# ablab/stringdecomposer

Hardware: AMD Instinct MI355X
Metric: decomposed read-bp/sec (whole node) at 12 monomers x 50kb reads (higher is better)
Workload: dtype u16

## Files before the change

include/sd_hip.h:

```cpp
#ifndef SD_HIP_H
#define SD_HIP_H

#include <stddef.h>
#include <stdint.h>

#ifdef __cplusplus
extern "C" {
#endif

#define SD_OK 0
#define SD_ERR_IO 2
#define SD_ERR_FORMAT 3
#define SD_ERR_PARAM 4
#define SD_ERR_EMPTY 6
#define SD_ERR_INTERNAL 7
#define SD_ERR_NO_DEVICE 8
#define SD_ERR_UNSUPPORTED 9
#define SD_ERR_HIP 10
#define SD_ERR_SYMBOL 255

typedef struct sd_params {
    int32_t ins, del, mismatch, match;
    int32_t part_size;
    int32_t overlap;
// ... 149 lines not shown

int sd_engine_load_reads(sd_engine* e, const char* const* read_seqs, const int64_t* read_lens,
                         int32_t n_reads, int64_t* n_chunks, char* errbuf, size_t errlen);

int sd_engine_load_reads_dev(sd_engine* e, const void* d_bases, const int64_t* read_off, const int64_t* read_lens,
                             int32_t n_reads, void* hip_stream, int64_t* n_chunks, char* errbuf, size_t errlen);

int sd_engine_run(sd_engine* e, void* hip_stream, char* errbuf, size_t errlen);

int sd_engine_fetch(sd_engine* e, sd_rec** recs, int64_t** rec_off, char* errbuf, size_t errlen);

int sd_engine_assemble(sd_engine* e, const sd_rec* recs, const int64_t* rec_off, sd_rec** rows,
                       int64_t** row_off, char* errbuf, size_t errlen);

int sd_engine_rows_dev(sd_engine* e, sd_rec* d_rows, int64_t cap_rows, int64_t* d_row_off, void* hip_stream, int64_t* n_rows,
                       char* errbuf, size_t errlen);

int sd_engine_timings(sd_engine* e, float ms[4]);

int sd_engine_info(sd_engine* e, int64_t info[8]);

int sd_plan_info(const sd_params* p, const char* const* mono_seqs, const int32_t* mono_lens, int32_t n_mono,
                 int64_t info[8], char* errbuf, size_t errlen);

typedef struct sd_stream sd_stream;
int sd_stream_create(sd_stream** out, const sd_params* p, const char* const* mono_seqs,
                     const int32_t* mono_lens, int32_t n_mono, int32_t sub_batches, char* errbuf,
                     size_t errlen);
void sd_stream_destroy(sd_stream* s);
int sd_stream_submit(sd_stream* s, const char* const* read_seqs, const int64_t* read_lens,
                     int32_t n_reads, char* errbuf, size_t errlen);
int sd_stream_submit_dev(sd_stream* s, const void* d_bases, const int64_t* read_off, const int64_t* read_lens,
                         int32_t n_reads, void* hip_stream, char* errbuf, size_t errlen);
int sd_stream_collect(sd_stream* s, sd_rec** rows, int64_t** row_off, int64_t* n_rows, char* errbuf,
                      size_t errlen);
int sd_stream_peek_dev(sd_stream* s, int32_t* n_reads, int64_t* max_rows, char* errbuf, size_t errlen);
int sd_stream_collect_dev(sd_stream* s, sd_rec* d_rows, int64_t cap_rows, int64_t* d_row_off, void* hip_stream,
                          int64_t* n_rows, char* errbuf, size_t errlen);
int sd_stream_stats(sd_stream* s, double out[16]);
int sd_stream_info(sd_stream* s, int64_t info[8]);

typedef struct sd_final_row {
    int32_t read;
    int64_t start, end;
    int32_t best, second, homo_best, homo_second;
    double ident, second_ident, homo_ident, homo_second_ident;
// ... 112 lines not shown
```

stringdecomposer_amd/csrc/sd_engine.hip:

```cpp
#include <hip/hip_runtime.h>

#include <fcntl.h>
#include <unistd.h>

#include <algorithm>
#include <atomic>
#include <condition_variable>
#include <deque>
#include <mutex>
#include <chrono>
#include <functional>
#include <cstdlib>
#include <cstring>
#include <memory>
#include <string>
#include <thread>
#include <vector>

#include "../../include/sd_hip.h"
#include "sd_convert.hpp"
#include "sd_ident.hpp"
#include "sd_nw.hpp"
#include "sd_device.hpp"
#include "sd_fast.hpp"
// ... 1066 lines not shown
        const int64_t L = (int64_t)e.tseq[j].size();
        int64_t run = 0, lanes_seen = 0;
        for (int64_t k = 0; k < L; ++k, ++x) {
            const uint32_t so = plan.slot_of[(size_t)x];
            const bool new_lane = k == 0 || (so & 127u) != (plan.slot_of[(size_t)x - 1] & 127u) || (so >> 16) != (plan.slot_of[(size_t)x - 1] >> 16);
            if (new_lane && k > 0) {
                if (lanes_seen == 0) min_first = std::min(min_first, run);
                max_lane = std::max(max_lane, run);
                ++lanes_seen;
                run = 0;
            }
            ++run;
        }
        if (lanes_seen == 0) min_first = std::min(min_first, run);
        max_lane = std::max(max_lane, run);
    }
    info[5] = min_first;
    info[6] = max_lane;
    info[7] = (int64_t)e.score_scale | ((int64_t)(plan.tr2_ok ? plan.tr2_qm : 0) << 16) | ((int64_t)(plan.tr2_ok ? plan.tr2_bound : 0) << 24) |
              ((int64_t)((plan.Hx >> 8) & 1) << 56);
    return SD_OK;
}

int sd_engine_create(sd_engine** out, const sd_params* p, const char* const* mono_seqs,
                     const int32_t* mono_lens, int32_t n_mono, char* errbuf, size_t errlen) {
    if (!out) return SD_ERR_PARAM;
    *out = nullptr;
    std::string err;
    int rc = validate_params(p, err);
    if (rc) { set_err(errbuf, errlen, err); return rc; }
    if (n_mono <= 0) { set_err(errbuf, errlen, "no monomers"); return SD_ERR_PARAM; }
    std::unique_ptr<sd_engine> e(new sd_engine);
    e->p = *p;
    apply_env_overrides(e->p);
    rc = host_templates(e.get(), *p, mono_seqs, mono_lens, n_mono, err);
    if (rc) { set_err(errbuf, errlen, err); return rc; }
    {
        const int w0 = (e->tlen[0] - 1) >> 6, h0 = ((e->tlen[0] - 1) >> 5) & 1;
        bool same = true;
        for (int j = 1; j < e->T; ++j) same = same && ((e->tlen[j] - 1) >> 6) == w0 && (((e->tlen[j] - 1) >> 5) & 1) == h0;
        e->filter_uniform = same && w0 == ((e->Lmax + 63) / 64) - 1 ? h0 : -1;
        if (e->p.reserved[1] & SD_FLAG_FILTER_GENERAL) e->filter_uniform = -1;
    }
    rc = check_score_range(*p, e->Lmax, err);
    if (rc) { set_err(errbuf, errlen, err); return rc; }

// ... 540 lines not shown
```

stringdecomposer_amd/csrc/sd_fast.hip:

```cpp
#include <hip/hip_runtime.h>

#include <algorithm>
#include <climits>
#include <cstdlib>
#include <type_traits>

#include "sd_fast.hpp"
#include "sd_fast_dev.hpp"
#include "sd_fast_launch.hpp"

namespace sd {

#ifndef SD_TRACE_MINW
#define SD_TRACE_MINW 7
#endif
#ifndef SD_TRACE_ADAPT
#define SD_TRACE_ADAPT 1
#endif
constexpr int trace_waves_per_group(int QK) { return QK <= 8 ? 4 : 1; }

template <int QK>
__global__ __launch_bounds__(64 * trace_waves_per_group(QK), (QK <= 4 ? SD_TRACE_MINW : QK <= 8 ? 2 : 1)) void sd_fast_trace(
    const ChunkDesc* __restrict__ chunks, int n_chunks, const uint32_t* __restrict__ bases2,
    const uint32_t* __restrict__ nmask, const uint32_t* __restrict__ slot_of,
// ... 425 lines not shown
            Bounds b2;
            const int fs = layout_for(c.first, b2);
            const int ops = cell_ops(c.first, fs);
            if (ops < best) { best = ops; P = c.first; split = c.second; plan.floor_slots = fs; bnd.swap(b2); }
        }
        plan.P = P;
        plan.P4 = (P + 3) & ~3;
    }
    for (int b = 0; b < 5; ++b) plan.floor_sym[b] = 1;
    plan.table_nonneg = std::min(sc.match, sc.mismatch) - sc.del - sc.ins >= 0;
    if (!plan.filter_only)
        for (int j = 0; j < T; ++j) {
            const std::string& sq = tseq[(size_t)j];
            const std::vector<int>& bj = bnd[(size_t)j];
            for (size_t u = 0; u + 1 < bj.size(); ++u)
                for (int b = 0; b < 5; ++b) {
                    int run = code_of(sq[(size_t)bj[u]]) == b ? sc.match : sc.mismatch;
                    for (int q = 1; bj[u] + q < bj[u + 1]; ++q) {
                        const int val = code_of(sq[(size_t)(bj[u] + q)]) == b ? sc.match : sc.mismatch;
                        if (val > run) { run = val; plan.floor_sym[b] = std::max(plan.floor_sym[b], q); }
                    }
                }
        }
    if (getenv("SD_PLAN_DEBUG"))
        std::fprintf(stderr, "[sd plan] P = %d: floor slots %d; per read symbol A C G T N: %d %d %d %d %d\n", P, plan.floor_slots,
                     plan.floor_sym[0], plan.floor_sym[1], plan.floor_sym[2], plan.floor_sym[3], plan.floor_sym[4]);
    plan.T = T;
    plan.split = split;
    plan.Lmax = Lmax;
    plan.Qk = (Lmax + 63) / 64;
    if (plan.Qk == 5) plan.Qk = 6;
    if (plan.Qk == 7) plan.Qk = 8;
    if (plan.Qk > 8) plan.Qk = plan.Qk <= 16 ? 16 : 32;
    plan.vlane0.assign((size_t)T, 0);
    int Vmax = 1;
    if (plan.tiled) {
        for (int j = 0; j < T; ++j) {
            plan.vlane0[(size_t)j] = tiled_v0[(size_t)j];
            Vmax = std::max(Vmax, ((int)tseq[(size_t)j].size() + P - 1) / P);
        }
        plan.bshift = 10;
    } else if (W > 1) {
        for (int j = 0; j < T; ++j) plan.vlane0[(size_t)j] = j;
        plan.bshift = 10;
    } else {
        int v = 0;
        for (int j = 0; j < T; ++j) {
            if (j == split) v = 64;
            plan.vlane0[(size_t)j] = v;
// ... 145 lines not shown
            plan.slot_of[(size_t)x] = (uint32_t)((slot << 7) | v);
            for (int b = 0; b < 5; ++b) {
                const int val = (cd == b ? sc.match : sc.mismatch) - sc.del - sc.ins;
                uint32_t& w = plan.table[(((size_t)b * (P4 / 4) + slot / 4) * 64 + lane) * 4 + (slot & 3)];
                put(w, plane, val);
            }
        }
    }
    if (allow_tr2) fast_plan_trace2(tseq, sc, plan);
    plan.ok = true;
    return true;
}

int64_t fast_ckpt_rows_total(const FastPlan& plan, std::vector<ChunkDesc>& chunks) {
    (void)plan;
    int64_t tot = 0;
    for (ChunkDesc& cd : chunks) {
        cd.pad = (uint32_t)tot;
        tot += (cd.n - 1) / FAST_R;
    }
    return tot;
}

uint32_t fast_fill_hx(const FastPlan& plan, int fl, int step) {
    uint32_t hx = plan.Hx;
    if (step > 0)
        for (int b = 0; b < 5; ++b) {
            uint32_t lv = 0;
            while (lv < 3 && fl - (int)(lv + 1) * step >= std::max(1, plan.floor_sym[b])) ++lv;
            hx |= lv << (22 + 2 * b);
        }
    return hx;
}

template <int... L> static int floor_level(const FastPlan& plan, PList<L...>) {
    for (int c : {L...})
        if (plan.floor_slots >= 1 && plan.floor_slots <= c && c + 2 < plan.P) return c;
    return 0;
}

static int multi_wave_fl(const FastPlan& plan) {
    return !plan.full_floor && floor_level(plan, PList<48>()) ? 48 : plan.P;
}

static void launch_fast_fill_full(const FastPlan& plan, hipStream_t st, const FillArgs& a, int grid, int nw, size_t lds, bool one) {
    with_p(FastP(), plan.P, [&](auto p) {
        constexpr int P = decltype(p)::value;
        with_bool(one, [&](auto on) {
            if (plan.f16) launch_narrow<P, CF_F16, P, decltype(on)::value, 0>(st, a, grid, nw, lds, plan.Hx);
            else launch_narrow<P, CF_I16, P, decltype(on)::value, 0>(st, a, grid, nw, lds, plan.Hx);
        });
    });
}

void launch_fast_fill(const FastPlan& plan, hipStream_t st, const FillArgs& a, size_t min_lds) {
// ... 71 lines not shown
```

stringdecomposer_amd/csrc/sd_fast.hpp:

```cpp
#pragma once

#include <hip/hip_runtime.h>

#include <cstdint>
#include <string>
#include <type_traits>
#include <vector>

#include "sd_device.hpp"

namespace sd {

constexpr int FAST_R = 32;
constexpr int FAST_REBASE = 128;
constexpr int FAST_LANE_WORDS = 8;

enum FastLaneConst {
    FLC_STARTMASK = 0,
    FLC_CONTMASK,
    FLC_ENDOFF,
    FLC_ROW0,
    FLC_TMPL,
    FLC_CONT2,
    FLC_ENDALL,
// ... 4 lines not shown
    bool ok = false;
    bool wide = false;
    bool f16 = false;
    bool u16 = false;
    int u16_lim = 0;
    int P = 0;
    int P4 = 0;
    int H = 0;
    uint32_t Hx = 0;
    int T = 0;
    int split = 0;
    int Lmax = 0;
    int Qk = 0;
    int waves = 1;
    bool tiled = false;
    bool filter_only = false;
    int bshift = 7;
    int rebase = FAST_REBASE;
    int range_bound = 0;
    bool full_floor = false;
    int floor_slots = 0;
    int floor_sym[5] = {0, 0, 0, 0, 0};
    bool table_nonneg = false;
    uint32_t bf8_match = 0, bf8_mismatch = 0;
    std::vector<int32_t> vlane0;
    std::vector<uint32_t> table;
    std::vector<uint32_t> lane_consts;
    std::vector<uint32_t> slot_of;
    std::vector<uint8_t> tcodes;
    std::vector<int32_t> end_vlane;
    std::vector<int32_t> end_off;
    bool tr2_ok = false;
    int tr2_qm = 0;
    int tr2_xlim = 0;
    int tr2_bound = 0;
    std::vector<uint32_t> tr2_tab;
};

void fast_plan_trace2(const std::vector<std::string>& tseq, ScoreArgs sc, FastPlan& plan);

inline bool fast_has_1bp(const FastPlan& plan) { return (plan.Hx >> 10) & 1; }

template <int... Vs> struct PList { static constexpr int v[] = {Vs...}; };
template <int... Vs, typename F> void with_p(PList<Vs...>, int v, F&& f) {
    (void)((v == Vs && (f(std::integral_constant<int, Vs>()), true)) || ...);
}
// ... 81 lines not shown
    const uint8_t* tcodes;
    const uint32_t* lane_consts;
    const int32_t* toff;
    const int32_t* tlen;
    ScoreArgs sc;
    const int32_t* B;
    const int32_t* argV;
    const uint32_t* ckpt;
    const int32_t* ckbase;
    DevRec* recs;
    int32_t* rec_cnt;
    int* queue;
    const int* order;
    int n_cu;
    const uint32_t* tr2_tab = nullptr;
    const uint16_t* klist = nullptr;
    const uint16_t* kpos = nullptr;
    const int32_t* nkept = nullptr;
    const uint32_t* lane_t = nullptr;
};

void launch_fast_fill(const FastPlan& plan, hipStream_t st, const FillArgs& a, size_t min_lds = 0);
void launch_fast_fill_compact(const FastPlan& plan, hipStream_t st, const FillArgs& a, int wb);
uint32_t fast_fill_hx(const FastPlan& plan, int fl, int step);

void launch_fast_fill_fl(const FastPlan& plan, hipStream_t st, const FillArgs& a, int grid, int nw, size_t lds, int fl);
void launch_fast_fill_fl_long(const FastPlan& plan, hipStream_t st, const FillArgs& a, int grid, int nw, size_t lds, int fl);
void launch_fast_fill_fl_u16(const FastPlan& plan, hipStream_t st, const FillArgs& a, int grid, int nw, size_t lds, int fl);
void launch_fast_fill_fl_long_u16(const FastPlan& plan, hipStream_t st, const FillArgs& a, int grid, int nw, size_t lds, int fl);
void launch_fast_fill_fl_u16s(const FastPlan& plan, hipStream_t st, const FillArgs& a, int grid, int nw, size_t lds, int fl);
void launch_fast_fill_fl_long_u16s(const FastPlan& plan, hipStream_t st, const FillArgs& a, int grid, int nw, size_t lds, int fl);
void launch_fast_fill_fl_i16(const FastPlan& plan, hipStream_t st, const FillArgs& a, int grid, int nw, size_t lds, int fl);
void launch_fast_fill_full_u16(const FastPlan& plan, hipStream_t st, const FillArgs& a, int grid, int nw, size_t lds, bool one);
void launch_fast_fill_wide(const FastPlan& plan, hipStream_t st, const FillArgs& a, int grid, size_t lds);
void launch_fast_fill_wide_fl(const FastPlan& plan, hipStream_t st, const FillArgs& a, int grid, size_t lds, int fl);
void launch_fast_fill_wn(const FastPlan& plan, hipStream_t st, const FillArgs& a, int grid, size_t lds);
void launch_fast_fill_wn_fl(const FastPlan& plan, hipStream_t st, const FillArgs& a, int grid, size_t lds);
void launch_fast_fill_wt(const FastPlan& plan, hipStream_t st, const FillArgs& a, int grid, size_t lds, int fl);
void launch_fast_fill_wn_i16(const FastPlan& plan, hipStream_t st, const FillArgs& a, int grid, size_t lds);
void launch_fast_fill_wt_i16(const FastPlan& plan, hipStream_t st, const FillArgs& a, int grid, size_t lds);
void launch_fast_fill_wn_compact(const FastPlan& plan, hipStream_t st, const FillArgs& a, int grid, int wb, size_t lds, int fl);
void launch_fast_fill_wt_compact(const FastPlan& plan, hipStream_t st, const FillArgs& a, int grid, int wb, size_t lds, int fl);

void launch_fast_trace(const FastPlan& plan, hipStream_t st, const TraceArgs& a);
void launch_fast_trace2(const FastPlan& plan, hipStream_t st, const TraceArgs& a);

}
// ... 1 lines not shown
```

stringdecomposer_amd/csrc/sd_fast_fill.hpp:

```cpp
#pragma once

#include <hip/hip_runtime.h>

#include <algorithm>
#include <climits>
#include <cstdlib>
#include <type_traits>

#include "sd_fast.hpp"
#include "sd_fast_dev.hpp"

namespace sd {

#define SD_FILL_NW_MAX 16
template <int P, bool RANKED, int CF, int FL = P, bool ONE = false, int FLS = 0>
__global__ __launch_bounds__(SD_FILL_NW_MAX * 64, 4) void sd_fast_fill(
    const ChunkDesc* __restrict__ chunks, int n_chunks, const uint32_t* __restrict__ bases2,
    const uint32_t* __restrict__ nmask, const uint32_t* __restrict__ table,
    const uint32_t* __restrict__ lane_consts, ScoreArgs sc, int Hx, int32_t* __restrict__ Bout,
    int32_t* __restrict__ argV, uint32_t* __restrict__ ckpt, int32_t* __restrict__ ckbase,
    int* __restrict__ queue, const int* __restrict__ order, const uint32_t* __restrict__ cendoff,
    const uint32_t* __restrict__ crank) {
    constexpr int P4 = (P + 3) & ~3;
    extern __shared__ __attribute__((aligned(16))) uint32_t lds[];
    constexpr int TBL = 5 * P4 * 64;
    constexpr bool F16 = CF == CF_F16, U16 = CF == CF_U16;
    using CO = CellOps<CF>;
    constexpr uint32_t NEGC = CO::NEG;
    for (int idx = threadIdx.x * 4; idx < TBL; idx += blockDim.x * 4) {
        uint4 q = *reinterpret_cast<const uint4*>(&table[idx]);
        if constexpr (F16) {
            q.x = CO::from_i16x2(q.x); q.y = CO::from_i16x2(q.y);
            q.z = CO::from_i16x2(q.z); q.w = CO::from_i16x2(q.w);
        }
        if constexpr (U16) {
            const uint32_t tm = lane_consts[((idx >> 2) & 63) * FAST_LANE_WORDS + FLC_TMPL];
            const int tpad = min(min(sc.match, sc.mismatch) - sc.del - sc.ins, 0);
            const int plo = (tm & 0xffffu) == 0xffffu ? 0 : tpad, phi = (tm >> 16) == 0xffffu ? 0 : tpad;
            auto cv = [&](uint32_t w) {
                const int lo = (int)(short)(w & 0xffffu), hi = (int)w >> 16;
                return spair(lo <= -30000 ? plo : lo, hi <= -30000 ? phi : hi);
            };
            q.x = cv(q.x); q.y = cv(q.y); q.z = cv(q.z); q.w = cv(q.w);
        }
        *reinterpret_cast<uint4*>(&lds[idx]) = q;
    }
    __syncthreads();

    const int wave = __builtin_amdgcn_readfirstlane((int)(threadIdx.x >> 6));
    const int nw = (int)(blockDim.x >> 6);
    const int lane = threadIdx.x & 63;
    (void)wave; (void)nw;
    const int H = Hx & 0xff;
    const bool bperm_ok = (Hx >> 8) & 1;
    FairShare fair;
    fair.init(reinterpret_cast<int*>(lds + TBL), wave, nw, lane, queue, n_chunks);
    ChunkSched sched;
    sched.init(queue, order, n_chunks);
    for (int c = sched.next(); c >= 0; c = sched.next()) {
    const ChunkDesc cd = chunks[c];
    const int n = cd.n;
    ReadStream rs;
    rs.init(bases2 + cd.woff, cd.noff >= 0 ? nmask + cd.noff : nullptr, n);
    bool bperm_scan = bperm_ok && (!fair.drained || ((Hx >> 9) & 1));

    const uint32_t* lc = lane_consts + lane * FAST_LANE_WORDS;
    const uint32_t startMask = lc[FLC_STARTMASK];
    const uint32_t contMask = lc[FLC_CONTMASK];
    const uint32_t cont2Mask = lc[FLC_CONT2];
    const uint32_t oneMask = ONE ? lc[FLC_ONE] : 0u;
    const uint32_t endOffPlan = lc[FLC_ENDOFF];
    constexpr bool HRED = F16 || U16;
    const uint32_t endOffRaw = pk_adds(RANKED ? cendoff[(size_t)c * 64 + lane] : lc[FLC_ENDALL], pack2(sc.del));
    const uint32_t endOff = HRED ? CO::from_i16x2(endOffRaw)
                                 : CO::from_i16x2(RANKED ? cendoff[(size_t)c * 64 + lane] : endOffPlan);
// ... 13 lines not shown
    int32_t* ckb = ckbase + cd.pad;

    uint32_t L[P];
    uint32_t tb[P4];
    uint32_t K = NEGC;
    int base = 0, Brel = 0, tp = 0;
    uint32_t bdel16 = 0;
    int accBV = 0;
    int flush_at = min(n, 64);

    typedef uint32_t u32x4_t __attribute__((ext_vector_type(4)));
    using lds_u4 = __attribute__((address_space(3))) const u32x4_t;
    const uint32_t lds_lane = (uint32_t)(uintptr_t)(__attribute__((address_space(3))) const uint32_t*)lds + lane * 16;
    auto load_table = [&](int r, uint32_t& after) {
        uint32_t addr = lds_lane + (uint32_t)(r * (P4 * 256));
        asm volatile("" : "+v"(addr), "+v"(after));
        lds_u4* t = (lds_u4*)(uintptr_t)addr;
#pragma unroll
        for (int c4 = 0; c4 < P4 / 4; ++c4) {
            const u32x4_t q = t[c4 * 64];
            tb[4 * c4 + 0] = q.x; tb[4 * c4 + 1] = q.y; tb[4 * c4 + 2] = q.z; tb[4 * c4 + 3] = q.w;
        }
    };
    const int idle4 = (Hx >> 16) << 2;
    int bp1 = (contMask & 0xffffu) ? (lane - 1) << 2 : idle4;
    int bp2 = (cont2Mask & 0xffffu) ? (lane - 2) << 2 : idle4;
    asm volatile("" : "+v"(bp1), "+v"(bp2));
    auto excl_scan = [&](uint32_t a) {
        uint32_t inc = a;
        if (bperm_scan) {
            inc = CO::mx(inc, (uint32_t)__builtin_amdgcn_ds_bpermute(bp1, (int)inc));
            inc = CO::mx(inc, (uint32_t)__builtin_amdgcn_ds_bpermute(bp2, (int)inc));
            return (uint32_t)__builtin_amdgcn_ds_bpermute(bp1, (int)inc);
        }
        if (H <= 4) {
            inc = CO::mx(inc, bfi(contMask, lane_up(inc, 1), NEGC));
            inc = CO::mx(inc, bfi(cont2Mask, lane_up(lane_up(inc, 1), 1), NEGC));
        } else {
            for (int h = 1; h < H; ++h) inc = CO::mx(a, bfi(contMask, lane_up(inc, 1), NEGC));
        }
        return bfi(contMask, lane_up(inc, 1), NEGC);
    };
    auto reduce_ends = [&](uint32_t Eend, int row) {
        if constexpr (HRED) {
            uint32_t val = CO::add(Eend, endOff);
            if constexpr (U16 && RANKED) val &= endMask;
            uint32_t m;
// ... 61 lines not shown
        const int v = mlo ? (__ffsll((long long)mlo) - 1) : (64 + __ffsll((long long)mhi) - 1);
        Brel = b + tp * sc.ins;
        const int slot = (row - 1) & 63;
        acc_put(accBV, (int)(((uint32_t)(base + Brel) << 7) | (uint32_t)v), slot);
        if (row == flush_at) {
            flush_at = min(n, row + 64);
            if (lane <= slot) Bc[row - slot + lane] = accBV;
        }
    };

    uint32_t pin = 0;
    load_table(rs.code(0), pin);
    rs.advance(0);
    if constexpr (U16) {
        L[0] = (tb[0] + row0adj + U16_BIAS2) & planeMask;
#pragma unroll
        for (int q = 1; q < P; ++q) L[q] = CO::mx(L[q - 1], (tb[q] + ins2 + U16_BIAS2) & planeMask);
    } else {
    L[0] = CO::add(tb[0], row0adj);
#pragma unroll
    for (int q = 1; q < P; ++q) L[q] = CO::mx(L[q - 1], CO::add(tb[q], ins2));
    }
    int rcur = rs.code(1);
    load_table(rcur, L[P - 1]);
    rs.advance(1);
    std::conditional_t<U16, U16Guard<P>, F16Guard<P>> guard;
    if constexpr (F16) {
        guard.start(L[P - 1], sc.guard_lim);
        guard.check_low(L);
    }
    if constexpr (U16) {
        guard.start(sc.guard_lim);
        guard.check_low(L, planeMask);
    }
    const uint32_t a0 = ONE ? bfi(oneMask, L[0], L[P - 1]) : L[P - 1];
    if constexpr (HRED) reduce_ends(a0, 1);
    K = excl_scan(a0);
    uint32_t Eend = CO::mx(a0, K);
    if constexpr (!HRED) reduce_ends(Eend, 1);

    for (int i = 1; i < n;) {
        if ((i & (FAST_R - 1)) == 0) {
            fair.update(n - i);
            bperm_scan = bperm_ok && (!fair.drained || ((Hx >> 9) & 1));
            if ((i & (127 >> ((Hx >> 11) & 1))) == 0) {
                if constexpr (F16)
// ... 33 lines not shown
            }
            const int q = (i / FAST_R) - 1;
#pragma unroll
            for (int s = 0; s < P; ++s) ck[(uint64_t)q * (P * 64) + s * 64] = CO::mx(L[s], K);
            if (lane == 0) ckb[q] = base + tp * sc.ins;
        }
        const int iend = min(n, (i | (FAST_R - 1)) + 1);
        for (; i < iend; ++i) {
        uint32_t KB;
        if constexpr (HRED) {
            asm("v_pk_max_f16 %0, %1, %2 op_sel_hi:[1,0]" : "=v"(KB) : "v"(K), "s"(bdel16));
            if constexpr (U16) KB &= planeMask;
        } else {
            KB = CO::mx(K, CO::splat(Brel + sc.del - tp * sc.ins));
        }
        const uint32_t w0 = U16 ? (L[0] & notStart) : bfi(startMask, NEGC, L[0]);
        uint32_t u_[P], v_[P], c_[P];
        uint32_t run = 0;
        if constexpr (HRED) {
            if constexpr (FLS > 0) {
                constexpr int FL3 = FL - 3 * FLS > 1 ? FL - 3 * FLS : 1;
                constexpr int FL2 = FL - 2 * FLS > FL3 ? FL - 2 * FLS : FL3;
                constexpr int FL1 = FL - FLS > FL2 ? FL - FLS : FL2;
                const int lv = (Hx >> (22 + 2 * rcur)) & 3;
#pragma unroll
                for (int q = 1; q <= FL3 && q < P; ++q) L[q - 1] = CO::mx(L[q - 1], KB);
                if (lv <= 2) {
#pragma unroll
                    for (int q = FL3 + 1; q <= FL2 && q < P; ++q) L[q - 1] = CO::mx(L[q - 1], KB);
                }
                if (lv <= 1) {
#pragma unroll
                    for (int q = FL2 + 1; q <= FL1 && q < P; ++q) L[q - 1] = CO::mx(L[q - 1], KB);
                }
                if (lv == 0) {
#pragma unroll
                    for (int q = FL1 + 1; q <= FL && q < P; ++q) L[q - 1] = CO::mx(L[q - 1], KB);
                }
            }
            const uint32_t w0f = FLS > 0 ? (U16 ? (L[0] & notStart) : bfi(startMask, NEGC, L[0])) : w0;
#pragma unroll
            for (int s = 0; s < P + 4; ++s) {
                if (s >= 4) {
                    const int q = s - 4;
                    L[q] = q == 0 ? CO::mx3(v_[0], w0f, K) : CO::mx3(L[q - 1], v_[q], L[q]);
                }
                if (s >= 2 && s - 2 < P) {
// ... 12 lines not shown
        } else {
#pragma unroll
        for (int s = 0; s < P + 3; ++s) {
            if (s >= 3) {
                const int q = s - 3;
                run = q == 0 ? c_[0] : pk_max(run, c_[q]);
                L[q] = run;
            }
            if (s >= 2 && s - 2 < P) {
                const int q = s - 2;
                c_[q] = pk_max(v_[q], q == 0 ? w0 : L[q]);
            }
            if (s >= 1 && s - 1 < P) {
                const int q = s - 1;
                v_[q] = pk_adds(u_[q], tb[q]);
            }
            if (s < P) {
                const int q = s;
                u_[q] = q == 0 ? KB : q <= FL ? pk_max(L[q - 1], KB) : L[q - 1];
            }
            __builtin_amdgcn_sched_barrier(0);
        }
        }
        rcur = rs.code(i + 1);
        load_table(rcur, L[P - 1]);
        rs.advance(i + 1);
        uint32_t a = HRED ? L[P - 1] : CO::mx(L[P - 1], K);
        if constexpr (ONE) a = bfi(oneMask, L[0], a);
        ++tp;
        if constexpr (HRED) {
            uint32_t t1 = 0;
            if (bperm_scan) t1 = (uint32_t)__builtin_amdgcn_ds_bpermute(bp1, (int)a);
            reduce_ends(a, i + 1);
            if (bperm_scan) {
                const uint32_t i1 = CO::mx(a, t1);
                const uint32_t i2 = CO::mx(i1, (uint32_t)__builtin_amdgcn_ds_bpermute(bp2, (int)i1));
                K = (uint32_t)__builtin_amdgcn_ds_bpermute(bp1, (int)i2);
            } else {
                K = excl_scan(a);
            }
        } else {
            K = excl_scan(a);
            Eend = CO::mx(a, K);
            reduce_ends(Eend, i + 1);
        }
        }
// ... 12 lines not shown
```

stringdecomposer_amd/csrc/sd_fast_fl.hip:

```cpp
#include "sd_fast_launch.hpp"

#ifndef SD_FL_CF
#define SD_FL_CF CF_F16
#define SD_FL_STEP 0
#define SD_FL_ENTRY launch_fast_fill_fl
#endif

namespace sd {

void SD_FL_ENTRY(const FastPlan& plan, hipStream_t st, const FillArgs& a, int grid, int nw, size_t lds, int fl) {
    const uint32_t hx = fast_fill_hx(plan, fl, SD_FL_STEP);
    with_p(FastFlP(), plan.P, [&](auto p) {
        with_p(FlLevels(), fl, [&](auto f) {
            launch_narrow<decltype(p)::value, SD_FL_CF, decltype(f)::value, false, SD_FL_STEP>(st, a, grid, nw, lds, hx);
        });
    });
}

}
```

stringdecomposer_amd/csrc/sd_fast_fl_long.hip:

```cpp
#include "sd_fast_launch.hpp"

#ifndef SD_FL_CF
#define SD_FL_CF CF_F16
#define SD_FL_STEP 0
#define SD_FL_ENTRY launch_fast_fill_fl_long
#endif

namespace sd {

void SD_FL_ENTRY(const FastPlan& plan, hipStream_t st, const FillArgs& a, int grid, int nw, size_t lds, int fl) {
    const uint32_t hx = fast_fill_hx(plan, fl, SD_FL_STEP);
    with_p(FastFlLongP(), plan.P, [&](auto p) {
        with_p(FlLongLevels(), fl, [&](auto f) {
            launch_narrow<decltype(p)::value, SD_FL_CF, decltype(f)::value, false, SD_FL_STEP>(st, a, grid, nw, lds, hx);
        });
    });
}

}
```

stringdecomposer_amd/csrc/sd_fast_launch.hpp:

```cpp
#pragma once

#include "sd_fast_fill.hpp"
#include "sd_fast_wide_fill.hpp"
#include "sd_fast_wn_fill.hpp"

namespace sd {

template <int P, int CF, int FL, bool ONE, int FLS>
void launch_narrow(hipStream_t st, const FillArgs& a, int grid, int nw, size_t lds, uint32_t hx) {
    with_bool(a.cendoff != nullptr, [&](auto rk) {
        constexpr bool RK = decltype(rk)::value;
        (void)hipFuncSetAttribute(reinterpret_cast<const void*>(&sd_fast_fill<P, RK, CF, FL, ONE, FLS>),
                                  hipFuncAttributeMaxDynamicSharedMemorySize, (int)lds);
        hipLaunchKernelGGL((sd_fast_fill<P, RK, CF, FL, ONE, FLS>), dim3(grid), dim3(nw * 64), lds, st, a.chunks, a.n_chunks,
                           a.bases2, a.nmask, a.table, a.lane_consts, a.sc, (int)hx, a.B, a.argV, a.ckpt, a.ckbase, a.queue,
                           a.order, a.cendoff, a.crank);
    });
}

template <int P, bool F16, int FL>
void launch_wide(hipStream_t st, const FillArgs& a, int grid, size_t lds) {
    with_bool(a.cendoff != nullptr, [&](auto rk) {
        constexpr bool RK = decltype(rk)::value;
        (void)hipFuncSetAttribute(reinterpret_cast<const void*>(&sd_fast_fill_wide<P, RK, F16, FL>),
                                  hipFuncAttributeMaxDynamicSharedMemorySize, (int)lds);
        hipLaunchKernelGGL((sd_fast_fill_wide<P, RK, F16, FL>), dim3(grid), dim3(512), lds, st, a.chunks, a.n_chunks, a.bases2,
                           a.nmask, a.table, a.lane_consts, a.sc, a.B, a.ckpt, a.ckbase, a.queue, a.order, a.cendoff, a.crank);
    });
}

template <int P, int FL, bool COMPACT, bool TILED, bool F16>
void launch_wn(const FastPlan& plan, hipStream_t st, const FillArgs& a, int grid, int nw, size_t lds) {
    auto go = [&](auto rk) {
        constexpr bool RK = decltype(rk)::value;
        (void)hipFuncSetAttribute(reinterpret_cast<const void*>(&sd_fast_fill_wn<P, RK, FL, COMPACT, TILED, F16>),
                                  hipFuncAttributeMaxDynamicSharedMemorySize, (int)lds);
        hipLaunchKernelGGL((sd_fast_fill_wn<P, RK, FL, COMPACT, TILED, F16>), dim3(grid), dim3(64 * nw), lds, st, a.chunks,
                           COMPACT ? 0 : a.n_chunks, a.bases2, a.nmask, COMPACT ? nullptr : a.table, a.lane_consts, a.sc,
// ... 12 lines not shown
```

stringdecomposer_amd/lib.py:

```python
import ctypes as C
import os
from collections import namedtuple

HERE = os.path.dirname(os.path.abspath(__file__))
LIB_PATH = os.environ.get("SD_HIP_LIB") or os.path.join(HERE, "csrc", "libsd_hip.so")

SD_OK = 0
SD_ERR_IO = 2
SD_ERR_FORMAT = 3
SD_ERR_PARAM = 4
SD_ERR_EMPTY = 6
SD_ERR_INTERNAL = 7
SD_ERR_NO_DEVICE = 8
SD_ERR_UNSUPPORTED = 9
SD_ERR_HIP = 10
SD_ERR_SYMBOL = 255

KERNEL_AUTO, KERNEL_GENERIC, KERNEL_FAST = 0, 1, 2

EXPORTS = [
    "sd_pipeline_logic_selftest",
    "sd_params_default", "sd_version", "sd_device_count", "sd_free", "sd_decompose_files",
    "sd_decompose", "sd_engine_create", "sd_engine_destroy", "sd_engine_load_reads",
    "sd_engine_run", "sd_engine_fetch", "sd_engine_assemble", "sd_engine_timings",
    "sd_engine_info", "sd_chunk_plan", "sd_seam_merge", "sd_format_rows", "sd_fasta_load",
    "sd_fasta_free", "sd_nw_identity_batch", "sd_identity_segments", "sd_chunk_table_size",
    "sd_decompose_chunk_range", "sd_assemble_tsv", "sd_release_cache", "sd_format_alt_rows",
    "sd_stream_create", "sd_stream_destroy", "sd_stream_submit", "sd_stream_collect", "sd_stream_stats",
    "sd_stream_info", "sd_pack_bases", "sd_identity_segments_dev", "sd_nw_release_cache", "sd_last_run_stats", "sd_guard_trips",
    "sd_run_files", "sd_convert_raw_tsv", "sd_decompose_files_range", "sd_assemble_files_tsv",
    "sd_host_stage_rates", "sd_run_files_range", "sd_plan_info", "sd_write_parts_selftest", "sd_convert_raw_tsv_range",
    "sd_write_records", "sd_read_records", "sd_records_free", "sd_records_to_raw_tsv", "sd_decompose_files_records",
    "sd_run_files_records",
    "sd_range_assemble_begin", "sd_range_assemble_begin_files", "sd_range_assemble_text", "sd_range_assemble_write",
    "sd_range_assemble_copy", "sd_range_assemble_stats", "sd_range_assemble_free", "sd_decompose_files_range_begin",
    "sd_range_assemble_records",
    "sd_run_files_devices", "sd_last_run_device_stats", "sd_multi_device_selftest",
    "sd_stream_create_final", "sd_stream_collect_final", "sd_stream_keys", "sd_stream_final_stats",
    "sd_stream_create_devices", "sd_stream_create_final_devices", "sd_stream_device_stats",
    "sd_profile_segments", "sd_profile_segments_dev", "sd_last_run_profile", "sd_stream_profile",
    "sd_stream_submit_dev", "sd_engine_load_reads_dev", "sd_pack_bases_dev", "sd_engine_filter_result",
    "sd_stream_peek_dev", "sd_stream_collect_dev", "sd_engine_rows_dev", "sd_seam_merge_dev", "sd_seam_pieces_selftest",
    "sd_stream_peek_final_dev", "sd_stream_collect_final_dev", "sd_final_select_dev", "sd_final_select_host",
    "sd_stream_profile_dev", "sd_stream_profile_stats", "sd_final_profile_dev", "sd_final_profile_host",
]


class SdError(RuntimeError):
    def __init__(self, code, msg):
        super().__init__("libsd_hip rc=%d: %s" % (code, msg))
        self.code = code
        self.msg = msg


class Params(C.Structure):
    _fields_ = [("ins", C.c_int32), ("del_", C.c_int32), ("mismatch", C.c_int32),
                ("match", C.c_int32), ("part_size", C.c_int32), ("overlap", C.c_int32),
                ("ed_thr", C.c_int32), ("threads", C.c_int32), ("device", C.c_int32),
                ("kernel", C.c_int32), ("max_batch_rows", C.c_int32), ("reserved", C.c_int32 * 5)]


class Rec(C.Structure):
    _fields_ = [("tmpl", C.c_int32), ("start", C.c_int32), ("end", C.c_int32),
                ("score", C.c_int32)]


class FinalRec(C.Structure):
# ... 31 lines not shown
                      "(or python -c 'import __graft_entry__ as g; g.build()')" % LIB_PATH)
    L = C.CDLL(LIB_PATH)
    P = C.POINTER
    L.sd_params_default.argtypes = [P(Params)]
    L.sd_version.restype = C.c_char_p
    L.sd_device_count.restype = C.c_int
    L.sd_free.argtypes = [C.c_void_p]
    L.sd_decompose_files.argtypes = [C.c_char_p, C.c_char_p, P(Params), C.c_char_p, C.c_char_p, C.c_size_t]
    L.sd_decompose.argtypes = [P(C.c_char_p), P(C.c_char_p), P(C.c_int64), C.c_int32, P(C.c_char_p),
                               P(C.c_char_p), P(C.c_int32), C.c_int32, P(Params), P(C.c_void_p),
                               P(C.c_size_t), C.c_char_p, C.c_size_t]
    L.sd_engine_create.argtypes = [P(C.c_void_p), P(Params), P(C.c_char_p), P(C.c_int32), C.c_int32,
                                   C.c_char_p, C.c_size_t]
    L.sd_engine_destroy.argtypes = [C.c_void_p]
    L.sd_engine_load_reads.argtypes = [C.c_void_p, P(C.c_char_p), P(C.c_int64), C.c_int32,
                                       P(C.c_int64), C.c_char_p, C.c_size_t]
    L.sd_engine_run.argtypes = [C.c_void_p, C.c_void_p, C.c_char_p, C.c_size_t]
    L.sd_engine_fetch.argtypes = [C.c_void_p, P(P(Rec)), P(P(C.c_int64)), C.c_char_p, C.c_size_t]
    L.sd_engine_assemble.argtypes = [C.c_void_p, P(Rec), P(C.c_int64), P(P(Rec)), P(P(C.c_int64)),
                                     C.c_char_p, C.c_size_t]
    L.sd_engine_timings.argtypes = [C.c_void_p, P(C.c_float)]
    L.sd_engine_info.argtypes = [C.c_void_p, P(C.c_int64)]
    L.sd_plan_info.argtypes = [P(Params), P(C.c_char_p), P(C.c_int32), C.c_int32, P(C.c_int64), C.c_char_p, C.c_size_t]
    L.sd_chunk_plan.restype = C.c_int32
    L.sd_chunk_plan.argtypes = [C.c_int64, C.c_int32, C.c_int32, P(C.c_int64), P(C.c_int32), C.c_int32]
    L.sd_seam_merge.restype = C.c_int32
    L.sd_seam_merge.argtypes = [P(Rec), C.c_int32]
    L.sd_format_rows.argtypes = [C.c_char_p, P(C.c_char_p), P(Rec), C.c_int32, P(C.c_void_p), P(C.c_size_t)]
    L.sd_fasta_load.argtypes = [C.c_char_p, P(Fasta), C.c_char_p, C.c_size_t]
    L.sd_fasta_free.argtypes = [P(Fasta)]
    L.sd_nw_identity_batch.argtypes = [P(C.c_char_p), P(C.c_int32), P(C.c_char_p), P(C.c_int32),
                                       C.c_int64, C.c_int32, P(C.c_int32), P(C.c_int32), P(C.c_int32)]
    L.sd_identity_segments.argtypes = [C.c_char_p, C.c_int64, C.c_void_p, C.c_void_p, C.c_int64,
                                       P(C.c_char_p), P(C.c_int32), C.c_int32, C.c_void_p, C.c_int32,
                                       C.c_int32, C.c_void_p, C.c_void_p, C.c_void_p]
    L.sd_identity_segments_dev.argtypes = [C.c_char_p, C.c_int64, C.c_void_p, C.c_void_p, C.c_int64,
                                           P(C.c_char_p), P(C.c_int32), C.c_int32, C.c_void_p, C.c_int32,
                                           C.c_int32, C.c_int32, C.c_void_p, C.c_void_p, C.c_void_p]
    L.sd_run_files.argtypes = [C.c_char_p, C.c_char_p, P(Params), C.c_char_p, C.c_char_p, C.c_char_p, C.c_int32,
                               C.c_int32, P(C.c_double), C.c_char_p, C.c_size_t]
    L.sd_run_files_range.argtypes = [C.c_char_p, C.c_char_p, P(Params), C.c_int32, C.c_int32, C.c_char_p, C.c_char_p,
                                     C.c_char_p, C.c_int32, C.c_int32, P(C.c_double), P(C.c_int64), C.c_char_p, C.c_size_t]
    L.sd_convert_raw_tsv.argtypes = [C.c_char_p, C.c_char_p, C.c_char_p, C.c_char_p, C.c_char_p, C.c_int32, C.c_int32,
                                     P(C.c_double), C.c_int32, C.c_int32, C.c_char_p, C.c_size_t]
    L.sd_decompose_files_range.argtypes = [C.c_char_p, C.c_char_p, P(Params), C.c_int32, C.c_int32, P(P(Rec)),
                                           P(P(C.c_int64)), P(C.c_int64), P(C.c_int64), P(C.c_int64), C.c_char_p,
# ... 129 lines not shown
    L = load()
    L.sd_guard_trips.restype = C.c_int64
    return int(L.sd_guard_trips())


def plan_info(mono_seqs, **kw):
    L = load()
    p = make_params(**kw)
    ms = [_b(s) for s in mono_seqs]
    ml = (C.c_int32 * max(len(ms), 1))(*[len(s) for s in ms])
    v = (C.c_int64 * 8)()
    err = C.create_string_buffer(4096)
    rc = L.sd_plan_info(C.byref(p), _strs(ms), ml, len(ms), v, err, 4096)
    if rc != SD_OK:
        raise SdError(rc, err.value.decode(errors="replace"))
    cells = {0: "int32", 1: "int16", 2: "f16", 9: "u16", 3: "int16/int8-table", 4: "f16/bf8-table", 5: "f16/bf8-codes x waves", 6: "f16/bf8-codes tiled x waves",
             7: "int16/int8-codes x waves", 8: "int16/int8-codes tiled x waves"}
    return {"family": {1: "generic", 2: "fast"}[v[0]], "cells_per_lane": v[1], "cells": cells.get(v[2], "?") if v[0] == 2 else "int32",
            "floor_slots": v[3], "waves": v[4] & 0xff, "range_bound": (v[4] >> 8) & 0xffffffff, "rebase": v[4] >> 40, "min_first_lane_cells": v[5], "max_lane_cells": v[6],
            "score_factor": v[7] & 0xffff, "trace_regs": (v[7] >> 16) & 0xff, "trace_bound": (v[7] >> 24) & 0xffffffff,
            "bperm_scan": bool((v[7] >> 56) & 1), "why": err.value.decode(errors="replace") if v[0] == 1 else ""}


def release_cache():
    load().sd_release_cache()


def device_count():
    return load().sd_device_count()


def decompose_files(reads_fa, monomers_fa, raw_tsv_out, **kw):
    L = load()
    p = make_params(**kw)
    err = C.create_string_buffer(4096)
    rc = L.sd_decompose_files(os.fsencode(reads_fa), os.fsencode(monomers_fa), C.byref(p),
                              os.fsencode(raw_tsv_out), err, 4096)
    if rc != SD_OK:
        raise SdError(rc, err.value.decode(errors="replace"))


def run_files(reads_fa, monomers_fa, raw_tsv_out, final_tsv_out, alt_tsv_out, min_identity=0, second_best=False,
              lr_coef=(-31.48494996, 0.41784018, 0.69186882), records_out=None, devices=None, profile=False, **kw):
    L = load()
    if profile:
        kw["flags"] = int(kw.get("flags", 0)) | FLAG_PROFILE
# ... 1284 lines not shown
```

Baseline: 3.838 billion.

## Refine fill floor levels by previous and current read symbol pair

Computes a per-pair (previous symbol, current symbol) table of floor levels at plan time and packs it into a 64-bit levels argument passed to the fill kernel. The kernel tracks the previous read code and indexes this table in place of the per-symbol level bits in Hx. The aim is to let more steps take the cheaper lower-level floor path, which skips max operations in the anti-diagonal update. The kernel carries an extra 64-bit argument and register, and the derivation relies on a new pair rule that holds only for certain score signs. A plan-inspection API and a Python wrapper are also added.

```diff
diff --git a/include/sd_hip.h b/include/sd_hip.h
--- a/include/sd_hip.h
+++ b/include/sd_hip.h
@@ -195,6 +195,10 @@
 
 int sd_plan_info(const sd_params* p, const char* const* mono_seqs, const int32_t* mono_lens, int32_t n_mono,
                  int64_t info[8], char* errbuf, size_t errlen);
+
+int sd_plan_floor_levels(const sd_params* p, const char* const* mono_seqs, const int32_t* mono_lens, int32_t n_mono,
+                         int32_t floor_sym[5], int32_t floor_pair[25], int32_t* lane_off, int32_t* lane_start, int64_t lane_cap,
+                         int64_t info[4], char* errbuf, size_t errlen);
 
 typedef struct sd_stream sd_stream;
 int sd_stream_create(sd_stream** out, const sd_params* p, const char* const* mono_seqs,
diff --git a/stringdecomposer_amd/csrc/sd_engine.hip b/stringdecomposer_amd/csrc/sd_engine.hip
--- a/stringdecomposer_amd/csrc/sd_engine.hip
+++ b/stringdecomposer_amd/csrc/sd_engine.hip
@@ -1112,6 +1112,47 @@
     return SD_OK;
 }
 
+int sd_plan_floor_levels(const sd_params* p, const char* const* mono_seqs, const int32_t* mono_lens, int32_t n_mono,
+                         int32_t floor_sym[5], int32_t floor_pair[25], int32_t* lane_off, int32_t* lane_start, int64_t lane_cap,
+                         int64_t info[4], char* errbuf, size_t errlen) {
+    std::string err;
+    int rc = validate_params(p, err);
+    if (rc) { set_err(errbuf, errlen, err); return rc; }
+    if (n_mono <= 0 || !mono_seqs || !mono_lens || !floor_sym || !floor_pair || !lane_off || !lane_start || !info) {
+        set_err(errbuf, errlen, "no monomers");
+        return SD_ERR_PARAM;
+    }
+    sd_engine e;
+    rc = host_templates(&e, *p, mono_seqs, mono_lens, n_mono, err);
+    if (rc) { set_err(errbuf, errlen, err); return rc; }
+    sd::FastPlan& plan = e.fplan;
+    std::string why;
+    e.p = *p;
+    apply_env_overrides(e.p);
+    const bool ok = plan_fast_family(e.p, e.tseq, e.sc, true, true, plan, why);
+    for (int i = 0; i < 4; ++i) info[i] = 0;
+    for (int i = 0; i < 5; ++i) floor_sym[i] = 0;
+    for (int i = 0; i < 25; ++i) floor_pair[i] = 0;
+    for (int j = 0; j <= e.T; ++j) lane_off[j] = 0;
+    info[0] = ok ? 2 : 1;
+    if (!ok) { set_err(errbuf, errlen, why); return SD_OK; }
+    info[1] = plan.P;
+    info[2] = plan.pair_rule ? 1 : 0;
+    for (int b = 0; b < 5; ++b) floor_sym[b] = plan.floor_sym[b];
+    for (int a = 0; a < 5; ++a)
+        for (int b = 0; b < 5; ++b) floor_pair[5 * a + b] = plan.floor_pair[a][b];
+    int64_t n = 0;
+    for (int j = 0; j < e.T; ++j) {
+        const std::vector<int32_t>& bj = plan.lane_bounds[(size_t)j];
+        for (size_t u = 0; u + 1 < bj.size(); ++u, ++n)
+            if (n < lane_cap) lane_start[n] = bj[u];
+        lane_off[j + 1] = (int32_t)n;
+    }
+    info[3] = n;
+    if (n > lane_cap) { set_err(errbuf, errlen, "lane_start too small"); return SD_ERR_PARAM; }
+    return SD_OK;
+}
+
 int sd_engine_create(sd_engine** out, const sd_params* p, const char* const* mono_seqs,
                      const int32_t* mono_lens, int32_t n_mono, char* errbuf, size_t errlen) {
     if (!out) return SD_ERR_PARAM;
diff --git a/stringdecomposer_amd/csrc/sd_fast.hip b/stringdecomposer_amd/csrc/sd_fast.hip
--- a/stringdecomposer_amd/csrc/sd_fast.hip
+++ b/stringdecomposer_amd/csrc/sd_fast.hip
@@ -471,9 +471,43 @@
                     }
                 }
         }
-    if (getenv("SD_PLAN_DEBUG"))
+    plan.pair_rule = plan.table_nonneg && sc.del <= 0 && !plan.filter_only;
+    for (int j = 0; j < T && plan.pair_rule; ++j) plan.pair_rule = ((int)tseq[(size_t)j].size() - 1) * sc.del + sc.del <= 0;
+    for (int a = 0; a < 5; ++a)
+        for (int b = 0; b < 5; ++b) plan.floor_pair[a][b] = plan.pair_rule && a < 4 ? 1 : plan.floor_sym[b];
+    if (plan.pair_rule) {
+        const int tmax = std::max(sc.match, sc.mismatch);
+        for (int j = 0; j < T; ++j) {
+            const std::string& sq = tseq[(size_t)j];
+            const std::vector<int>& bj = bnd[(size_t)j];
+            for (size_t u = 0; u + 1 < bj.size(); ++u)
+                for (int b = 0; b < 5; ++b) {
+                    int run = code_of(sq[(size_t)bj[u]]) == b ? sc.match : sc.mismatch;
+                    bool top[4] = {false, false, false, false};
+                    for (int q = 1; bj[u] + q < bj[u + 1]; ++q) {
+                        const int cp = code_of(sq[(size_t)(bj[u] + q - 1)]);
+                        for (int a = 0; a < 4; ++a) top[a] = top[a] || (cp == a ? sc.match : sc.mismatch) == tmax;
+                        const int val = code_of(sq[(size_t)(bj[u] + q)]) == b ? sc.match : sc.mismatch;
+                        if (val > run) {
+                            run = val;
+                            for (int a = 0; a < 4; ++a)
+                                if (!top[a]) plan.floor_pair[a][b] = std::max(plan.floor_pair[a][b], q);
+                        }
+                    }
+                }
+        }
+    }
+    plan.lane_bounds.assign((size_t)T, std::vector<int32_t>());
+    if (!plan.filter_only)
+        for (int j = 0; j < T; ++j) plan.lane_bounds[(size_t)j].assign(bnd[(size_t)j].begin(), bnd[(size_t)j].end());
+    if (getenv("SD_PLAN_DEBUG")) {
         std::fprintf(stderr, "[sd plan] P = %d: floor slots %d; per read symbol A C G T N: %d %d %d %d %d\n", P, plan.floor_slots,
                      plan.floor_sym[0], plan.floor_sym[1], plan.floor_sym[2], plan.floor_sym[3], plan.floor_sym[4]);
+        for (int a = 0; a < 5; ++a)
+            std::fprintf(stderr, "[sd plan]   after %c: %d %d %d %d %d%s\n", "ACGTN"[a], plan.floor_pair[a][0], plan.floor_pair[a][1],
+                         plan.floor_pair[a][2], plan.floor_pair[a][3], plan.floor_pair[a][4],
+                         a == 0 ? (plan.pair_rule ? "   (by previous and current symbol)" : "   (pair rule off: per-symbol levels)") : "");
+    }
     plan.T = T;
     plan.split = split;
     plan.Lmax = Lmax;
@@ -665,15 +699,18 @@
     return tot;
 }
 
-uint32_t fast_fill_hx(const FastPlan& plan, int fl, int step) {
-    uint32_t hx = plan.Hx;
-    if (step > 0)
+uint64_t fast_fill_levels(const FastPlan& plan, int fl, int step) {
+    uint64_t levels = 0;
+    if (step <= 0) return levels;
+    const bool by_symbol = getenv("SD_FILL_SYMBOL_LEVEL") != nullptr;
+    for (int a = 0; a < 5; ++a)
         for (int b = 0; b < 5; ++b) {
-            uint32_t lv = 0;
-            while (lv < 3 && fl - (int)(lv + 1) * step >= std::max(1, plan.floor_sym[b])) ++lv;
-            hx |= lv << (22 + 2 * b);
-        }
-    return hx;
+            const int need = std::max(1, by_symbol ? plan.floor_sym[b] : plan.floor_pair[a][b]);
+            uint64_t lv = 0;
+            while (lv < 3 && fl - (int)(lv + 1) * step >= need) ++lv;
+            levels |= lv << (2 * (5 * a + b));
+        }
+    return levels;
 }
 
 template <int... L> static int floor_level(const FastPlan& plan, PList<L...>) {
diff --git a/stringdecomposer_amd/csrc/sd_fast.hpp b/stringdecomposer_amd/csrc/sd_fast.hpp
--- a/stringdecomposer_amd/csrc/sd_fast.hpp
+++ b/stringdecomposer_amd/csrc/sd_fast.hpp
@@ -50,6 +50,9 @@
     int floor_slots = 0;
     int floor_sym[5] = {0, 0, 0, 0, 0};
     bool table_nonneg = false;
+    int floor_pair[5][5] = {};
+    bool pair_rule = false;
+    std::vector<std::vector<int32_t>> lane_bounds;
     uint32_t bf8_match = 0, bf8_mismatch = 0;
     std::vector<int32_t> vlane0;
     std::vector<uint32_t> table;
@@ -177,7 +180,7 @@
 
 void launch_fast_fill(const FastPlan& plan, hipStream_t st, const FillArgs& a, size_t min_lds = 0);
 void launch_fast_fill_compact(const FastPlan& plan, hipStream_t st, const FillArgs& a, int wb);
-uint32_t fast_fill_hx(const FastPlan& plan, int fl, int step);
+uint64_t fast_fill_levels(const FastPlan& plan, int fl, int step);
 
 void launch_fast_fill_fl(const FastPlan& plan, hipStream_t st, const FillArgs& a, int grid, int nw, size_t lds, int fl);
 void launch_fast_fill_fl_long(const FastPlan& plan, hipStream_t st, const FillArgs& a, int grid, int nw, size_t lds, int fl);
diff --git a/stringdecomposer_amd/csrc/sd_fast_fill.hpp b/stringdecomposer_amd/csrc/sd_fast_fill.hpp
--- a/stringdecomposer_amd/csrc/sd_fast_fill.hpp
+++ b/stringdecomposer_amd/csrc/sd_fast_fill.hpp
@@ -17,7 +17,7 @@
 __global__ __launch_bounds__(SD_FILL_NW_MAX * 64, 4) void sd_fast_fill(
     const ChunkDesc* __restrict__ chunks, int n_chunks, const uint32_t* __restrict__ bases2,
     const uint32_t* __restrict__ nmask, const uint32_t* __restrict__ table,
-    const uint32_t* __restrict__ lane_consts, ScoreArgs sc, int Hx, int32_t* __restrict__ Bout,
+    const uint32_t* __restrict__ lane_consts, ScoreArgs sc, uint32_t Hx, unsigned long long levels, int32_t* __restrict__ Bout,
     int32_t* __restrict__ argV, uint32_t* __restrict__ ckpt, int32_t* __restrict__ ckbase,
     int* __restrict__ queue, const int* __restrict__ order, const uint32_t* __restrict__ cendoff,
     const uint32_t* __restrict__ crank) {
@@ -50,7 +50,7 @@
     const int wave = __builtin_amdgcn_readfirstlane((int)(threadIdx.x >> 6));
     const int nw = (int)(blockDim.x >> 6);
     const int lane = threadIdx.x & 63;
-    (void)wave; (void)nw;
+    (void)wave; (void)nw; (void)levels;
     const int H = Hx & 0xff;
     const bool bperm_ok = (Hx >> 8) & 1;
     FairShare fair;
@@ -110,7 +110,7 @@
             tb[4 * c4 + 0] = q.x; tb[4 * c4 + 1] = q.y; tb[4 * c4 + 2] = q.z; tb[4 * c4 + 3] = q.w;
         }
     };
-    const int idle4 = (Hx >> 16) << 2;
+    const int idle4 = (int)(((Hx >> 16) & 63u) << 2);
     int bp1 = (contMask & 0xffffu) ? (lane - 1) << 2 : idle4;
     int bp2 = (cont2Mask & 0xffffu) ? (lane - 2) << 2 : idle4;
     asm volatile("" : "+v"(bp1), "+v"(bp2));
@@ -218,6 +218,8 @@
     for (int q = 1; q < P; ++q) L[q] = CO::mx(L[q - 1], CO::add(tb[q], ins2));
     }
     int rcur = rs.code(1);
+    int rprev = 4;
+    (void)rprev;
     load_table(rcur, L[P - 1]);
     rs.advance(1);
     std::conditional_t<U16, U16Guard<P>, F16Guard<P>> guard;
@@ -297,7 +299,7 @@
                 constexpr int FL3 = FL - 3 * FLS > 1 ? FL - 3 * FLS : 1;
                 constexpr int FL2 = FL - 2 * FLS > FL3 ? FL - 2 * FLS : FL3;
                 constexpr int FL1 = FL - FLS > FL2 ? FL - FLS : FL2;
-                const int lv = (Hx >> (22 + 2 * rcur)) & 3;
+                const int lv = (int)(levels >> (2 * (5 * rprev + rcur))) & 3;
 #pragma unroll
                 for (int q = 1; q <= FL3 && q < P; ++q) L[q - 1] = CO::mx(L[q - 1], KB);
                 if (lv <= 2) {
@@ -356,6 +358,7 @@
             __builtin_amdgcn_sched_barrier(0);
         }
         }
+        rprev = rcur;
         rcur = rs.code(i + 1);
         load_table(rcur, L[P - 1]);
         rs.advance(i + 1);
diff --git a/stringdecomposer_amd/csrc/sd_fast_fl.hip b/stringdecomposer_amd/csrc/sd_fast_fl.hip
--- a/stringdecomposer_amd/csrc/sd_fast_fl.hip
+++ b/stringdecomposer_amd/csrc/sd_fast_fl.hip
@@ -9,10 +9,10 @@
 namespace sd {
 
 void SD_FL_ENTRY(const FastPlan& plan, hipStream_t st, const FillArgs& a, int grid, int nw, size_t lds, int fl) {
-    const uint32_t hx = fast_fill_hx(plan, fl, SD_FL_STEP);
+    const uint64_t levels = fast_fill_levels(plan, fl, SD_FL_STEP);
     with_p(FastFlP(), plan.P, [&](auto p) {
         with_p(FlLevels(), fl, [&](auto f) {
-            launch_narrow<decltype(p)::value, SD_FL_CF, decltype(f)::value, false, SD_FL_STEP>(st, a, grid, nw, lds, hx);
+            launch_narrow<decltype(p)::value, SD_FL_CF, decltype(f)::value, false, SD_FL_STEP>(st, a, grid, nw, lds, plan.Hx, levels);
         });
     });
 }
diff --git a/stringdecomposer_amd/csrc/sd_fast_fl_long.hip b/stringdecomposer_amd/csrc/sd_fast_fl_long.hip
--- a/stringdecomposer_amd/csrc/sd_fast_fl_long.hip
+++ b/stringdecomposer_amd/csrc/sd_fast_fl_long.hip
@@ -9,10 +9,10 @@
 namespace sd {
 
 void SD_FL_ENTRY(const FastPlan& plan, hipStream_t st, const FillArgs& a, int grid, int nw, size_t lds, int fl) {
-    const uint32_t hx = fast_fill_hx(plan, fl, SD_FL_STEP);
+    const uint64_t levels = fast_fill_levels(plan, fl, SD_FL_STEP);
     with_p(FastFlLongP(), plan.P, [&](auto p) {
         with_p(FlLongLevels(), fl, [&](auto f) {
-            launch_narrow<decltype(p)::value, SD_FL_CF, decltype(f)::value, false, SD_FL_STEP>(st, a, grid, nw, lds, hx);
+            launch_narrow<decltype(p)::value, SD_FL_CF, decltype(f)::value, false, SD_FL_STEP>(st, a, grid, nw, lds, plan.Hx, levels);
         });
     });
 }
diff --git a/stringdecomposer_amd/csrc/sd_fast_launch.hpp b/stringdecomposer_amd/csrc/sd_fast_launch.hpp
--- a/stringdecomposer_amd/csrc/sd_fast_launch.hpp
+++ b/stringdecomposer_amd/csrc/sd_fast_launch.hpp
@@ -7,13 +7,13 @@
 namespace sd {
 
 template <int P, int CF, int FL, bool ONE, int FLS>
-void launch_narrow(hipStream_t st, const FillArgs& a, int grid, int nw, size_t lds, uint32_t hx) {
+void launch_narrow(hipStream_t st, const FillArgs& a, int grid, int nw, size_t lds, uint32_t hx, uint64_t levels = 0) {
     with_bool(a.cendoff != nullptr, [&](auto rk) {
         constexpr bool RK = decltype(rk)::value;
         (void)hipFuncSetAttribute(reinterpret_cast<const void*>(&sd_fast_fill<P, RK, CF, FL, ONE, FLS>),
                                   hipFuncAttributeMaxDynamicSharedMemorySize, (int)lds);
         hipLaunchKernelGGL((sd_fast_fill<P, RK, CF, FL, ONE, FLS>), dim3(grid), dim3(nw * 64), lds, st, a.chunks, a.n_chunks,
-                           a.bases2, a.nmask, a.table, a.lane_consts, a.sc, (int)hx, a.B, a.argV, a.ckpt, a.ckbase, a.queue,
+                           a.bases2, a.nmask, a.table, a.lane_consts, a.sc, hx, levels, a.B, a.argV, a.ckpt, a.ckbase, a.queue,
                            a.order, a.cendoff, a.crank);
     });
 }
diff --git a/stringdecomposer_amd/lib.py b/stringdecomposer_amd/lib.py
--- a/stringdecomposer_amd/lib.py
+++ b/stringdecomposer_amd/lib.py
@@ -43,6 +43,7 @@
     "sd_stream_peek_dev", "sd_stream_collect_dev", "sd_engine_rows_dev", "sd_seam_merge_dev", "sd_seam_pieces_selftest",
     "sd_stream_peek_final_dev", "sd_stream_collect_final_dev", "sd_final_select_dev", "sd_final_select_host",
     "sd_stream_profile_dev", "sd_stream_profile_stats", "sd_final_profile_dev", "sd_final_profile_host",
+    "sd_plan_floor_levels",
 ]
 
 
@@ -120,6 +121,8 @@
     L.sd_engine_timings.argtypes = [C.c_void_p, P(C.c_float)]
     L.sd_engine_info.argtypes = [C.c_void_p, P(C.c_int64)]
     L.sd_plan_info.argtypes = [P(Params), P(C.c_char_p), P(C.c_int32), C.c_int32, P(C.c_int64), C.c_char_p, C.c_size_t]
+    L.sd_plan_floor_levels.argtypes = [P(Params), P(C.c_char_p), P(C.c_int32), C.c_int32, P(C.c_int32), P(C.c_int32), P(C.c_int32),
+                                       P(C.c_int32), C.c_int64, P(C.c_int64), C.c_char_p, C.c_size_t]
     L.sd_chunk_plan.restype = C.c_int32
     L.sd_chunk_plan.argtypes = [C.c_int64, C.c_int32, C.c_int32, P(C.c_int64), P(C.c_int32), C.c_int32]
     L.sd_seam_merge.restype = C.c_int32
@@ -295,6 +298,25 @@
             "bperm_scan": bool((v[7] >> 56) & 1), "why": err.value.decode(errors="replace") if v[0] == 1 else ""}
 
 
+def plan_floor_levels(mono_seqs, **kw):
+    L = load()
+    p = make_params(**kw)
+    ms = [_b(s) for s in mono_seqs]
+    ml = (C.c_int32 * max(len(ms), 1))(*[len(s) for s in ms])
+    T, cap = 2 * len(ms), 2 * sum(len(s) for s in ms) + 1
+    sym, pair = (C.c_int32 * 5)(), (C.c_int32 * 25)()
+    off, start = (C.c_int32 * (T + 1))(), (C.c_int32 * cap)()
+    v = (C.c_int64 * 4)()
+    err = C.create_string_buffer(4096)
+    rc = L.sd_plan_floor_levels(C.byref(p), _strs(ms), ml, len(ms), sym, pair, off, start, cap, v, err, 4096)
+    if rc != SD_OK:
+        raise SdError(rc, err.value.decode(errors="replace"))
+    return {"family": {1: "generic", 2: "fast"}[v[0]], "cells_per_lane": v[1], "pair_rule": bool(v[2]),
+            "floor_sym": list(sym), "floor_pair": [list(pair[5 * a:5 * a + 5]) for a in range(5)],
+            "lane_starts": [list(start[off[j]:off[j + 1]]) for j in range(T)],
+            "why": err.value.decode(errors="replace") if v[0] == 1 else ""}
+
+
 def release_cache():
     load().sd_release_cache()
 
```

New measurement: 3.918 billion, median of 6. 1.02x the previous value.
